# grailbio/bigslice

Hardware: AMD Instinct MI355X
Metric: rows/sec (whole node) Reshuffle+Reduce group-by (higher is better)
Workload: dtype int64; 1 GPU; model=Reshuffle+Reduce group-by-sum (BASELINE config 3), rows_total=125000000, rows_per_gpu=125000000, distinct_keys=1000000, global_batch=125000000, parallelism=dp1, device=cuda:0

## Files before the change

bigslice_amd/csrc/ext.hip:

```cpp

#include <torch/extension.h>

#include <ATen/hip/HIPContext.h>
#include <hip/hip_runtime.h>

#include <vector>

#include "hash_partition.hip"
#include "groupby.hip"
#include "groupby_part.hip"
#include "sort.hip"
#include "radix.hip"
#include "runs.hip"
#include "runs_multi.hip"
#include "vecagg.hip"
#include "strings.hip"
#include "expr.hip"
#include "tokenize.hip"
#include "groupby_multi.hip"

namespace {

#define HIP_CHECK(expr)                                              \
  do {                                                               \
// ... 187 lines not shown
  TORCH_CHECK(cap > 0 && (cap & (cap - 1)) == 0, "capacity must be 2^k");
  TORCH_CHECK(tkeys.is_cuda() && tkeys.is_contiguous() &&
              tkeys.scalar_type() == torch::kInt64);
  for (const auto& tab : tabs)
    TORCH_CHECK(tab.is_cuda() && tab.is_contiguous() &&
                tab.size(0) == cap + 1);
  TORCH_CHECK(flags.is_cuda() && flags.is_contiguous() &&
              flags.scalar_type() == torch::kInt32 && flags.numel() >= 2);
  return cap;
}

uint32_t bucket_shift(int64_t cap, int64_t nbuckets) {
  TORCH_CHECK(cap > 0 && (cap & (cap - 1)) == 0 && cap <= (int64_t(1) << 31),
              "capacity must be 2^k");
  TORCH_CHECK(nbuckets >= 2 && nbuckets <= GBP_MAX_BUCKETS &&
                  (nbuckets & (nbuckets - 1)) == 0 && nbuckets <= cap,
              "nbuckets must be a power of two in [2, ", GBP_MAX_BUCKETS,
              "] and at most the capacity");
  uint32_t shift = 0;
  while ((cap >> shift) > nbuckets) ++shift;
  return shift;
}

void groupby_insert(torch::Tensor keys, std::vector<torch::Tensor> vals,
                    std::vector<int64_t> aggs, torch::Tensor tkeys,
                    std::vector<torch::Tensor> tabs, torch::Tensor flags,
                    int64_t max_probes) {
  TORCH_CHECK(keys.is_cuda() && keys.scalar_type() == torch::kInt64);
  keys = keys.contiguous();
  int64_t n = keys.size(0);
  if (n == 0) return;
  int64_t cap = table_cap(tkeys, tabs, flags);
  ValCols vc = make_val_cols(vals, tabs, aggs);
  int blocks = (int)std::min<int64_t>((n + THREADS - 1) / THREADS, 32768);
  hipLaunchKernelGGL(k_groupby_insert, dim3(blocks), dim3(THREADS), 0,
                     current_stream(), keys.data_ptr<int64_t>(), n, vc,
                     tkeys.data_ptr<int64_t>(), cap, GB_HASH_SEED,
                     flags.data_ptr<int32_t>(),
                     flags.data_ptr<int32_t>() + 1, max_probes);
  HIP_CHECK(hipGetLastError());
}

torch::Tensor slot_pids(torch::Tensor keys, int64_t cap,
                        int64_t nparts) {
  TORCH_CHECK(keys.is_cuda() && keys.scalar_type() == torch::kInt64);
  keys = keys.contiguous();
  int64_t n = keys.size(0);
  auto pids = torch::empty({n}, keys.options().dtype(torch::kInt32));
  int blocks = (int)std::min<int64_t>((n + THREADS - 1) / THREADS, 32768);
  hipLaunchKernelGGL(k_slot_pids, dim3(blocks), dim3(THREADS), 0,
                     current_stream(), keys.data_ptr<int64_t>(), n, cap,
                     (int32_t)nparts, GB_HASH_SEED,
                     pids.data_ptr<int32_t>());
  HIP_CHECK(hipGetLastError());
  return pids;
}

void groupby_insert_lds(torch::Tensor keys, torch::Tensor vals,
                        torch::Tensor tkeys, torch::Tensor tab,
                        torch::Tensor flags, int64_t max_probes,
                        int64_t target_blocks) {
  TORCH_CHECK(keys.is_cuda() && keys.scalar_type() == torch::kInt64);
  TORCH_CHECK(vals.scalar_type() == torch::kInt64);
  keys = keys.contiguous();
  vals = vals.contiguous();
  int64_t n = keys.size(0);
  if (n == 0) return;
  int64_t cap = table_cap(tkeys, {tab}, flags);
  if (target_blocks <= 0) target_blocks = 32768;
  int64_t nblocks = std::min<int64_t>((n + THREADS - 1) / THREADS,
                                      target_blocks);
  int64_t rpb = 0;
  hipLaunchKernelGGL(k_groupby_insert_sum_i64_lds, dim3((uint32_t)nblocks),
                     dim3(THREADS), 0, current_stream(),
                     keys.data_ptr<int64_t>(), vals.data_ptr<int64_t>(), n,
                     tkeys.data_ptr<int64_t>(),
                     (long long*)tab.data_ptr<int64_t>(), cap, GB_HASH_SEED,
                     flags.data_ptr<int32_t>(),
                     flags.data_ptr<int32_t>() + 1, max_probes, rpb,
                     (int32_t)1, (uint32_t*)nullptr);
  HIP_CHECK(hipGetLastError());
}

std::tuple<torch::Tensor, torch::Tensor> part_scatter_impl(
    const torch::Tensor& keys, const torch::Tensor& vals, int64_t cap,
    int64_t nbuckets) {
  int64_t n = keys.size(0);
  TORCH_CHECK(n > 0 && n < (int64_t(1) << 31), "1 <= rows < 2^31");
  const uint32_t shift = bucket_shift(cap, nbuckets);
  const uint32_t seed = GB_HASH_SEED;
  const uint32_t mask = (uint32_t)(cap - 1);
  const uint32_t nb = (uint32_t)nbuckets;
  const int64_t ntiles = (n + GBP_SCATTER_ROWS - 1) / GBP_SCATTER_ROWS;
  auto opts32 = keys.options().dtype(torch::kInt32);
  auto hist = torch::empty({ntiles * nbuckets}, opts32);
  auto totals = torch::empty({nbuckets}, opts32);
  auto pairs = torch::empty({n, 2}, keys.options());
  auto stream = current_stream();
  hipLaunchKernelGGL(k_gbp_hist, dim3((uint32_t)ntiles), dim3(GBP_THREADS),
                     0, stream, keys.data_ptr<int64_t>(), n, nb, seed, mask,
                     shift, (uint32_t*)hist.data_ptr<int32_t>());
  HIP_CHECK(hipGetLastError());
  hipLaunchKernelGGL(k_gbp_offsets, dim3((nb + 63) / 64),
                     dim3(GBP_OFF_THREADS), 0, stream,
                     (uint32_t*)hist.data_ptr<int32_t>(), ntiles, nb,
                     (uint32_t*)totals.data_ptr<int32_t>());
  HIP_CHECK(hipGetLastError());
  const int64_t per_xcd = (ntiles + 7) / 8;
  hipLaunchKernelGGL(k_gbp_scatter, dim3((uint32_t)(8 * per_xcd)),
                     dim3(GBP_THREADS), 0, stream,
                     keys.data_ptr<int64_t>(), vals.data_ptr<int64_t>(), n,
                     ntiles, nb, seed, mask, shift,
                     (const uint32_t*)hist.data_ptr<int32_t>(),
                     (const uint32_t*)totals.data_ptr<int32_t>(),
                     (GbPair*)pairs.data_ptr<int64_t>());
  HIP_CHECK(hipGetLastError());
  return {pairs, totals};
}

void launch_gbp_aggregate(const torch::Tensor& pairs,
                          const torch::Tensor& tkeys,
                          const torch::Tensor& tab,
                          const torch::Tensor& flags, int64_t cap,
                          int64_t max_probes) {
  const int64_t n = pairs.size(0);
  const int64_t ntiles = (n + GBP_TILE_ROWS - 1) / GBP_TILE_ROWS;
  hipLaunchKernelGGL(k_gbp_aggregate, dim3((uint32_t)ntiles),
                     dim3(GBP_THREADS), 0, current_stream(),
                     (const GbPair*)pairs.data_ptr<int64_t>(), n,
                     tkeys.data_ptr<int64_t>(),
                     (long long*)tab.data_ptr<int64_t>(), cap, GB_HASH_SEED,
                     flags.data_ptr<int32_t>(),
                     flags.data_ptr<int32_t>() + 1, max_probes);
  HIP_CHECK(hipGetLastError());
}

torch::Tensor part_owned_impl(const torch::Tensor& pairs,
                              const torch::Tensor& totals,
                              const torch::Tensor& tkeys,
                              const torch::Tensor& tab,
                              const torch::Tensor& flags,
                              int64_t max_probes) {
  const int64_t n = pairs.size(0);
  const int64_t cap = table_cap(tkeys, {tab}, flags);
  const int64_t nbuckets = totals.size(0);
  TORCH_CHECK(n > 0 && n < (int64_t(1) << 31), "1 <= rows < 2^31");
  const uint32_t shift = bucket_shift(cap, nbuckets);
  const int64_t S = cap / nbuckets;
  TORCH_CHECK(S <= GBP_LDS_SLOTS, "owned pass needs capacity / nbuckets <= ",
              GBP_LDS_SLOTS);
  TORCH_CHECK((uintptr_t)tkeys.data_ptr() % 16 == 0 &&
                  (uintptr_t)tab.data_ptr() % 16 == 0,
              "table must be 16-byte aligned");
  const uint32_t nb = (uint32_t)nbuckets;
  const uint32_t seed = GB_HASH_SEED;
  auto clean = torch::empty({nbuckets}, totals.options());
  auto todo = torch::empty({nbuckets, 2}, totals.options());
  auto stream = current_stream();
  HIP_CHECK(hipFuncSetAttribute(
      (const void*)k_gbp_owned, hipFuncAttributeMaxDynamicSharedMemorySize,
      16 * GBP_LDS_SLOTS));
  hipLaunchKernelGGL(k_gbp_owned, dim3(nb), dim3(GBP_THREADS),
                     (size_t)(16 * S), stream,
                     (GbPair*)pairs.data_ptr<int64_t>(), n,
                     (const uint32_t*)totals.data_ptr<int32_t>(), nb,
                     (uint32_t)S, tkeys.data_ptr<int64_t>(),
                     (long long*)tab.data_ptr<int64_t>(), seed, max_probes,
                     (uint32_t*)clean.data_ptr<int32_t>(),
                     (uint2*)todo.data_ptr<int32_t>());
  HIP_CHECK(hipGetLastError());
  const int64_t ntiles = (n + GBP_TILE_ROWS - 1) / GBP_TILE_ROWS;
  hipLaunchKernelGGL(k_gbp_cleanup, dim3((uint32_t)ntiles),
                     dim3(GBP_THREADS), 0, stream,
                     (const GbPair*)pairs.data_ptr<int64_t>(), n,
                     tkeys.data_ptr<int64_t>(),
                     (long long*)tab.data_ptr<int64_t>(), cap, seed,
                     flags.data_ptr<int32_t>(),
                     flags.data_ptr<int32_t>() + 1, max_probes,
                     (const uint2*)todo.data_ptr<int32_t>(), nb, shift);
  HIP_CHECK(hipGetLastError());
  return clean;
}

void groupby_insert_part(torch::Tensor keys, torch::Tensor vals,
                         torch::Tensor tkeys, torch::Tensor tab,
                         torch::Tensor flags, int64_t max_probes,
                         int64_t nbuckets, int64_t owned) {
  TORCH_CHECK(keys.is_cuda() && keys.scalar_type() == torch::kInt64);
  TORCH_CHECK(vals.scalar_type() == torch::kInt64 &&
              vals.size(0) == keys.size(0));
  TORCH_CHECK(tab.scalar_type() == torch::kInt64);
  keys = keys.contiguous();
  vals = vals.contiguous();
  if (keys.size(0) == 0) return;
  int64_t cap = table_cap(tkeys, {tab}, flags);
  auto parts = part_scatter_impl(keys, vals, cap, nbuckets);
  const torch::Tensor& pairs = std::get<0>(parts);
  if (owned)
    part_owned_impl(pairs, std::get<1>(parts), tkeys, tab, flags,
                    max_probes);
  else
    launch_gbp_aggregate(pairs, tkeys, tab, flags, cap, max_probes);
}

std::tuple<torch::Tensor, torch::Tensor> groupby_part_scatter(
    torch::Tensor keys, torch::Tensor vals, int64_t cap,
    int64_t nbuckets) {
  TORCH_CHECK(keys.is_cuda() && keys.scalar_type() == torch::kInt64);
  TORCH_CHECK(vals.scalar_type() == torch::kInt64 &&
              vals.size(0) == keys.size(0));
  return part_scatter_impl(keys.contiguous(), vals.contiguous(), cap,
                           nbuckets);
}

void groupby_part_aggregate(torch::Tensor pairs, torch::Tensor tkeys,
                            torch::Tensor tab, torch::Tensor flags,
                            int64_t max_probes) {
  TORCH_CHECK(pairs.is_cuda() && pairs.scalar_type() == torch::kInt64 &&
              pairs.is_contiguous() && pairs.dim() == 2 &&
              pairs.size(1) == 2);
  if (pairs.size(0) == 0) return;
  TORCH_CHECK(tab.scalar_type() == torch::kInt64);
  launch_gbp_aggregate(pairs, tkeys, tab, flags,
                       table_cap(tkeys, {tab}, flags), max_probes);
}

torch::Tensor groupby_part_owned(torch::Tensor pairs, torch::Tensor totals,
                                 torch::Tensor tkeys, torch::Tensor tab,
                                 torch::Tensor flags, int64_t max_probes) {
  TORCH_CHECK(pairs.is_cuda() && pairs.scalar_type() == torch::kInt64 &&
              pairs.is_contiguous() && pairs.dim() == 2 &&
              pairs.size(1) == 2);
  TORCH_CHECK(totals.is_cuda() && totals.scalar_type() == torch::kInt32 &&
              totals.is_contiguous() && totals.dim() == 1);
  TORCH_CHECK(tab.scalar_type() == torch::kInt64);
  return part_owned_impl(pairs, totals, tkeys, tab, flags, max_probes);
}

std::vector<torch::Tensor> groupby_compact(torch::Tensor tkeys,
                                           std::vector<torch::Tensor> tabs,
                                           torch::Tensor cursor) {
  int64_t cap = tkeys.size(0) - 1;
  CompactCols cc;
  cc.n = (int)tabs.size();
  std::vector<torch::Tensor> out;
  auto out_keys = torch::empty({cap}, tkeys.options());
  out.push_back(out_keys);
  for (size_t c = 0; c < tabs.size(); ++c) {
    out.push_back(torch::empty({cap}, tabs[c].options()));
    cc.tab[c] = {tabs[c].data_ptr(), dtype_code(tabs[c])};
    cc.out[c] = {out[c + 1].data_ptr(), dtype_code(tabs[c])};
  }
  int64_t spb = (cap + 2047) / 2048;
  if (spb < THREADS) spb = THREADS;
  int blocks = (int)((cap + spb - 1) / spb);
  hipLaunchKernelGGL(k_groupby_compact, dim3(blocks), dim3(THREADS), 0,
                     current_stream(), tkeys.data_ptr<int64_t>(), cap, spb,
                     cc, out_keys.data_ptr<int64_t>(),
                     (unsigned long long*)cursor.data_ptr());
  HIP_CHECK(hipGetLastError());
  return out;
}


#define GBM_LAUNCH(kernel, nk, blocks, ...)                              \
  do {                                                                   \
    switch (nk) {                                                        \
      case 2:                                                            \
        hipLaunchKernelGGL(kernel<2>, dim3(blocks), dim3(THREADS), 0,    \
                           current_stream(), __VA_ARGS__);               \
        break;                                                           \
      case 3:                                                            \
        hipLaunchKernelGGL(kernel<3>, dim3(blocks), dim3(THREADS), 0,    \
                           current_stream(), __VA_ARGS__);               \
        break;                                                           \
      case 4:                                                            \
        hipLaunchKernelGGL(kernel<4>, dim3(blocks), dim3(THREADS), 0,    \
                           current_stream(), __VA_ARGS__);               \
        break;                                                           \
      default:                                                           \
        hipLaunchKernelGGL(kernel<0>, dim3(blocks), dim3(THREADS), 0,    \
                           current_stream(), __VA_ARGS__);               \
    }                                                                    \
    HIP_CHECK(hipGetLastError());                                        \
  } while (0)

uint64_t gbm_fp_mask(int64_t fp_bits) {
  TORCH_CHECK(fp_bits >= 1 && fp_bits <= 64, "fp_bits must be in [1, 64]");
  return fp_bits == 64 ? ~uint64_t(0) : (uint64_t(1) << fp_bits) - 1;
}

int64_t gbm_batch_keys(MkCols& kc, const std::vector<torch::Tensor>& keys) {
  TORCH_CHECK(keys.size() >= 2 && (int)keys.size() <= MAX_KEY_COLS,
              "2..", MAX_KEY_COLS, " key columns supported");
  kc.n = (int)keys.size();
// ... 715 lines not shown
    else if (J == 2) launch(k_expr<true, 2>);
    else launch(k_expr<true, 1>);
  } else {
    if (J == 4) launch(k_expr<false, 4>);
    else if (J == 2) launch(k_expr<false, 2>);
    else launch(k_expr<false, 1>);
  }
  HIP_CHECK(hipGetLastError());
  return outs;
}

std::vector<torch::Tensor> tokenize_bytes(torch::Tensor data,
                                          torch::Tensor offsets,
                                          std::vector<uint64_t> mask4,
                                          bool with_rows) {
  TORCH_CHECK(data.is_cuda() && data.is_contiguous() && data.dim() == 1 &&
              data.scalar_type() == torch::kUInt8,
              "tokenize_bytes: contiguous uint8 device data required");
  TORCH_CHECK(offsets.is_cuda() && offsets.is_contiguous() &&
              offsets.dim() == 1 && offsets.size(0) >= 1 &&
              offsets.scalar_type() == torch::kInt64,
              "tokenize_bytes: contiguous int64 device offsets required");
  TORCH_CHECK(mask4.size() == 4, "tokenize_bytes: mask4 has 4 words");
  const int64_t total = data.size(0);
  const int64_t n = offsets.size(0) - 1;
  TORCH_CHECK(total < (1ll << 31),
              "tokenize_bytes: total bytes must be below 2^31");
  TORCH_CHECK(n > 0 || total == 0, "tokenize_bytes: bytes without rows");
  auto i64 = offsets.options();
  if (total == 0) {
    std::vector<torch::Tensor> out = {torch::empty({0}, data.options()),
                                      torch::zeros({1}, i64)};
    if (with_rows) out.push_back(torch::empty({0}, i64));
    return out;
  }
  if (((uintptr_t)data.data_ptr<uint8_t>() & 15) != 0) data = data.clone();
  const TokMask m{mask4[0], mask4[1], mask4[2], mask4[3]};
  auto stream = current_stream();
  const int64_t ntiles = (total + TOK_TILE - 1) / TOK_TILE;
  auto counts = torch::empty({ntiles, 2}, i64.dtype(torch::kInt32));
  hipLaunchKernelGGL(k_tok_count, dim3((int)ntiles), dim3(TOK_BLOCK), 0,
                     stream, data.data_ptr<uint8_t>(), total,
                     offsets.data_ptr<int64_t>(), n, m,
                     (unsigned int*)counts.data_ptr<int32_t>());
  HIP_CHECK(hipGetLastError());
  auto incl = at::cumsum(counts.view(torch::kInt64).flatten(), 0);
  const uint64_t totals = (uint64_t)incl[ntiles - 1].item<int64_t>();
  const int64_t nkept = (int64_t)(totals & 0xFFFFFFFFull);
  const int64_t ntok = (int64_t)(totals >> 32);
  auto out_data = torch::empty({nkept}, data.options());
  auto out_offsets = torch::empty({ntok + 1}, i64);
  torch::Tensor tok_row;
  if (with_rows) tok_row = torch::empty({ntok}, i64);
  hipLaunchKernelGGL(k_tok_write, dim3((int)ntiles), dim3(TOK_BLOCK), 0,
                     stream, data.data_ptr<uint8_t>(), total,
                     offsets.data_ptr<int64_t>(), n, m,
                     (const unsigned int*)incl.data_ptr<int64_t>(), nkept,
                     ntok,
                     out_data.data_ptr<uint8_t>(),
                     out_offsets.data_ptr<int64_t>(),
                     with_rows ? tok_row.data_ptr<int64_t>() : nullptr);
  HIP_CHECK(hipGetLastError());
  std::vector<torch::Tensor> out = {out_data, out_offsets};
  if (with_rows) out.push_back(tok_row);
  return out;
}

}

PYBIND11_MODULE(TORCH_EXTENSION_NAME, m) {
  m.def("hash_columns", &hash_columns, "murmur3 row hash (K3)");
  m.def("hash_partition", &hash_partition,
        "fused hash+histogram+scatter partitioner (K4)");
  m.def("scatter_by_partition", &scatter_by_partition,
        "scatter rows by precomputed partition ids");
  m.def("groupby_insert", &groupby_insert,
        "hash-aggregate insert pass (K9)");
  m.def("groupby_insert_lds", &groupby_insert_lds,
        "two-level LDS+global insert (int64 sum)");
  m.def("groupby_insert_part", &groupby_insert_part,
        "partitioned LDS pre-aggregating insert (single i64 sum)",
        py::arg("keys"), py::arg("vals"), py::arg("tkeys"), py::arg("tab"),
        py::arg("flags"), py::arg("max_probes"), py::arg("nbuckets"),
        py::arg("owned") = 0);
  m.def("groupby_part_owned", &groupby_part_owned,
        "owner + cleanup passes of the partitioned insert; returns clean");
  m.attr("GBP_OWN_LIMIT") = (int64_t)GBP_OWN_LIMIT;
  m.def("groupby_part_scatter", &groupby_part_scatter,
        "bucket scatter of the partitioned insert");
  m.def("groupby_part_aggregate", &groupby_part_aggregate,
        "aggregate pass of the partitioned insert");
  m.attr("GBP_TILE_ROWS") = (int64_t)GBP_TILE_ROWS;
  m.attr("GBP_LDS_SLOTS") = (int64_t)GBP_LDS_SLOTS;
  m.attr("GBP_MAX_BUCKETS") = (int64_t)GBP_MAX_BUCKETS;
  m.def("groupby_compact", &groupby_compact,
        "hash-aggregate table compaction (K9)");
  m.def("groupby_mk_insert", &groupby_mk_insert,
        "multi-column-key hash-aggregate insert: claim + accumulate (K21)",
        py::arg("keys"), py::arg("vals"), py::arg("aggs"), py::arg("tags"),
        py::arg("kcols"), py::arg("tabs"), py::arg("flags"),
        py::arg("max_probes"), py::arg("fp_bits") = 64);
  m.def("groupby_mk_claim", &groupby_mk_claim,
        "launch 1 of groupby_mk_insert; returns the rows' slots");
  m.def("groupby_mk_accum", &groupby_mk_accum,
        "launch 2 of groupby_mk_insert");
  m.def("groupby_mk_fingerprint", &groupby_mk_fingerprint,
        "the tuple fingerprint groupby_mk_insert claims slots by",
        py::arg("keys"), py::arg("fp_bits") = 64);
  m.attr("MAX_KEY_COLS") = (int64_t)MAX_KEY_COLS;
  m.attr("MAX_COLS") = (int64_t)MAX_COLS;
  m.def("agg_identity", &agg_identity, "aggregation identity fill");
  m.def("radix_argsort", &radix_argsort, "device radix argsort (K6)");
  m.def("radix_sort_keys", &radix_sort_keys, "device radix key sort",
        py::arg("keys"), py::arg("probe") = true);
  m.def("runs_sorted", &runs_sorted,
        "run boundaries of sorted keys (K18)");
  m.def("runs_multi", &runs_multi,
        "run boundaries of lexicographically sorted key columns (K22)");
  m.attr("MRUNS_TILE_ROWS") = (int64_t)MRUNS_TILE;
  m.def("lex_searchsorted", &lex_searchsorted,
        "searchsorted over lexicographically sorted tuples (K22)",
        py::arg("sorted_cols"), py::arg("query_cols"),
        py::arg("right") = false);
  m.def("segment_reduce_runs", &segment_reduce_runs,
        "int64 segmented reduce with precomputed runs (K16 fast path)");
  m.def("runs_guard", &runs_guard,
        "(count, max run length) of a runs_sorted result");
  m.def("segment_reduce_sorted", &segment_reduce_sorted,
        "typed reduce-by-key over sorted pairs (K16; deterministic)");
  m.def("hash_bytes", &hash_bytes,
        "murmur3-32 over varlen byte rows (K17, device strings)");
  m.def("hash_bytes64", &hash_bytes64,
        "64-bit two-seed murmur3 dictionary ids (K17)");
  m.def("colsum16", &colsum16,
        "vector-aggregate experiment: [N,16] f32 colsum, VALU vs MFMA");
  m.def("radix_sort_kv", &radix_sort_kv,
        "direct (key, 8-byte value) radix sort");
  m.def("slot_pids", &slot_pids, "table-slot-range partition ids");
  m.def("expr_apply", &expr_apply,
        "fused Map/Filter expression interpreter (K13)");
  m.def("tokenize_bytes", &tokenize_bytes,
        "split BYTES rows into tokens on a delimiter set (K20)");
  m.attr("TOKENIZE_TILE_BYTES") = (int64_t)TOK_TILE;
}
```

bigslice_amd/csrc/groupby_part.hip:

```cpp

#include <hip/hip_runtime.h>

#include "columns.h"

#define GBP_THREADS 512
#define GBP_SCATTER_ROWS 4096
#define GBP_TILE_ROWS 8192
#define GBP_LDS_SLOTS 4096
#define GBP_LDS_BITS 12
#define GBP_LDS_PROBES 8
#define GBP_MAX_BUCKETS 1024

struct __attribute__((aligned(16))) GbPair {
  long long k;
  long long v;
};

__device__ __forceinline__ uint32_t gbp_bucket(long long k, uint32_t seed,
                                               uint32_t mask,
                                               uint32_t shift) {
  if (k == GB_SENTINEL) return 0;
  return (mm3_u64((uint64_t)k, seed) & mask) >> shift;
}

extern "C" __global__ __launch_bounds__(GBP_THREADS) void k_gbp_hist(
    const int64_t* keys, int64_t n, uint32_t nb, uint32_t seed,
    uint32_t mask, uint32_t shift, uint32_t* hist) {
  __shared__ uint32_t lh[GBP_MAX_BUCKETS];
  for (uint32_t b = threadIdx.x; b < nb; b += GBP_THREADS) lh[b] = 0;
  __syncthreads();
  const int64_t base = (int64_t)blockIdx.x * GBP_SCATTER_ROWS;
#pragma unroll
  for (int j = 0; j < GBP_SCATTER_ROWS / GBP_THREADS; ++j) {
    const int64_t i = base + j * GBP_THREADS + threadIdx.x;
    if (i < n) atomicAdd(&lh[gbp_bucket(keys[i], seed, mask, shift)], 1u);
  }
  __syncthreads();
  uint32_t* row = hist + (int64_t)blockIdx.x * nb;
  for (uint32_t b = threadIdx.x; b < nb; b += GBP_THREADS) row[b] = lh[b];
}

#define GBP_OFF_THREADS 1024
#define GBP_OFF_WAVES (GBP_OFF_THREADS / 64)

extern "C" __global__ __launch_bounds__(GBP_OFF_THREADS) void k_gbp_offsets(
    uint32_t* hist, int64_t ntiles, uint32_t nb, uint32_t* totals) {
  __shared__ uint32_t wsum[GBP_OFF_WAVES][64];
  const int lane = threadIdx.x & 63;
  const int w = threadIdx.x >> 6;
  const uint32_t col = blockIdx.x * 64 + lane;
  const bool ok = col < nb;
  const int64_t chunk = (ntiles + GBP_OFF_WAVES - 1) / GBP_OFF_WAVES;
  const int64_t t0 = min((int64_t)w * chunk, ntiles);
  const int64_t t1 = min(t0 + chunk, ntiles);
  uint32_t s = 0;
  if (ok) {
#pragma unroll 8
    for (int64_t t = t0; t < t1; ++t) s += hist[t * nb + col];
  }
  wsum[w][lane] = s;
  __syncthreads();
  uint32_t run = 0;
  for (int w2 = 0; w2 < w; ++w2) run += wsum[w2][lane];
  if (w == GBP_OFF_WAVES - 1 && ok) totals[col] = run + s;
  if (!ok) return;
  int64_t t = t0;
  for (; t + 8 <= t1; t += 8) {
    uint32_t v[8];
#pragma unroll
    for (int j = 0; j < 8; ++j) v[j] = hist[(t + j) * nb + col];
#pragma unroll
    for (int j = 0; j < 8; ++j) {
      hist[(t + j) * nb + col] = run;
      run += v[j];
    }
  }
  for (; t < t1; ++t) {
    const uint32_t v = hist[t * nb + col];
    hist[t * nb + col] = run;
    run += v;
  }
}

__device__ __forceinline__ void gbp_block_scan(uint32_t* a, uint32_t nb,
                                               uint32_t* wtmp) {
  const uint32_t i0 = 2 * threadIdx.x;
  const uint32_t x0 = i0 < nb ? a[i0] : 0;
  const uint32_t x1 = i0 + 1 < nb ? a[i0 + 1] : 0;
  const uint32_t s = x0 + x1;
  const int lane = threadIdx.x & 63;
  const int w = threadIdx.x >> 6;
  uint32_t run = s;
  for (int off = 1; off < 64; off <<= 1) {
    const uint32_t up = __shfl_up(run, off);
    if (lane >= off) run += up;
  }
  if (lane == 63) wtmp[w] = run;
  __syncthreads();
  uint32_t base = 0;
  for (int w2 = 0; w2 < w; ++w2) base += wtmp[w2];
  const uint32_t excl = base + run - s;
  if (i0 < nb) a[i0] = excl;
  if (i0 + 1 < nb) a[i0 + 1] = excl + x0;
  __syncthreads();
}

extern "C" __global__ __launch_bounds__(GBP_THREADS) void k_gbp_scatter(
    const int64_t* keys, const int64_t* vals, int64_t n, int64_t ntiles,
    uint32_t nb, uint32_t seed, uint32_t mask, uint32_t shift,
    const uint32_t* hist, const uint32_t* totals, GbPair* out) {
  __shared__ GbPair stage[GBP_SCATTER_ROWS];
  __shared__ uint32_t lstart[GBP_MAX_BUCKETS];
  __shared__ uint32_t delta[GBP_MAX_BUCKETS];
  __shared__ uint32_t wtmp[GBP_THREADS / 64];
  const int64_t per_xcd = (ntiles + 7) / 8;
  const int64_t tile = (int64_t)(blockIdx.x & 7) * per_xcd + (blockIdx.x >> 3);
  if (tile >= ntiles) return;
  for (uint32_t b = threadIdx.x; b < nb; b += GBP_THREADS) {
    lstart[b] = 0;
    delta[b] = totals[b];
  }
  __syncthreads();
  constexpr int R = GBP_SCATTER_ROWS / GBP_THREADS;
  const int64_t base = tile * GBP_SCATTER_ROWS;
  const uint32_t cnt = (uint32_t)min((int64_t)GBP_SCATTER_ROWS, n - base);
  long long k[R], v[R];
  uint32_t br[R];
#pragma unroll
  for (int j = 0; j < R; ++j) {
    const uint32_t p = j * GBP_THREADS + threadIdx.x;
    if (p < cnt) {
      k[j] = keys[base + p];
      v[j] = vals[base + p];
    }
  }
#pragma unroll
  for (int j = 0; j < R; ++j) {
    const uint32_t p = j * GBP_THREADS + threadIdx.x;
    if (p < cnt) {
      const uint32_t b = gbp_bucket(k[j], seed, mask, shift);
      br[j] = (b << 16) | atomicAdd(&lstart[b], 1u);
    }
  }
  __syncthreads();
  gbp_block_scan(lstart, nb, wtmp);
  gbp_block_scan(delta, nb, wtmp);
#pragma unroll
  for (int j = 0; j < R; ++j) {
    const uint32_t p = j * GBP_THREADS + threadIdx.x;
    if (p < cnt) {
      GbPair pr;
      pr.k = k[j];
      pr.v = v[j];
      stage[lstart[br[j] >> 16] + (br[j] & 0xffffu)] = pr;
    }
  }
  const uint32_t* hrow = hist + tile * nb;
  for (uint32_t b = threadIdx.x; b < nb; b += GBP_THREADS)
    delta[b] += hrow[b] - lstart[b];
  __syncthreads();
  for (uint32_t p = threadIdx.x; p < cnt; p += GBP_THREADS) {
    const GbPair pr = stage[p];
    const uint32_t b = gbp_bucket(pr.k, seed, mask, shift);
    const uint32_t d = delta[b] + p;
    if (d < n) out[d] = pr;
  }
}

__device__ __forceinline__ bool gbp_lds_add(long long k, long long v,
                                            long long* lk, long long* lv,
                                            uint32_t seed) {
  uint32_t h = (mm3_u64((uint64_t)k, seed) * 0x9e3779b1u) >>
               (32 - GBP_LDS_BITS);
  for (int p = 0; p < GBP_LDS_PROBES; ++p) {
    long long cur = lk[h];
    if (cur == GB_SENTINEL) {
      const long long prev = atomicCAS((unsigned long long*)&lk[h],
                                       (unsigned long long)GB_SENTINEL,
                                       (unsigned long long)k);
      cur = (prev == GB_SENTINEL) ? k : prev;
    }
    if (cur == k) {
      atomicAdd((unsigned long long*)&lv[h], (unsigned long long)v);
      return true;
    }
    h = (h + 1) & (GBP_LDS_SLOTS - 1);
  }
  return false;
}

template <bool CLEAN>
__device__ __forceinline__ void gbp_aggregate_tile(
    const GbPair* pairs, int64_t n, int64_t* tkeys, long long* tab,
    int64_t cap, uint32_t seed, int32_t* sentinel_seen, int32_t* overflow,
    int64_t max_probes, const uint2* todo, uint32_t nb, uint32_t shift) {
  __shared__ long long lk[GBP_LDS_SLOTS];
  __shared__ long long lv[GBP_LDS_SLOTS];
  __shared__ uint32_t lend[CLEAN ? GBP_MAX_BUCKETS : 1];
  __shared__ uint32_t hull[2];
  const uint64_t gmask = (uint64_t)cap - 1;
  const int64_t base = (int64_t)blockIdx.x * GBP_TILE_ROWS;
  int64_t first = base, last = n;
  if constexpr (CLEAN) {
    const uint32_t t0 = (uint32_t)base;
    const uint32_t t1 = (uint32_t)min(base + GBP_TILE_ROWS, n);
    if (threadIdx.x == 0) {
      hull[0] = t1;
      hull[1] = t0;
    }
    __syncthreads();
    for (uint32_t b = threadIdx.x; b < nb; b += GBP_THREADS) {
      const uint2 se = todo[b];
      lend[b] = se.y;
      if (se.y > se.x && se.x < t1 && se.y > t0) {
        atomicMin(&hull[0], max(se.x, t0));
        atomicMax(&hull[1], min(se.y, t1));
      }
    }
    __syncthreads();
    first = hull[0];
    last = hull[1];
    if (first >= last) return;
    if (last - first <= GBP_THREADS) {
      const int64_t i = first + threadIdx.x;
      if (i < last) {
        const GbPair pr = pairs[i];
        if (i < (int64_t)lend[gbp_bucket(pr.k, seed, (uint32_t)gmask, shift)])
          gb_global_insert_sum(pr.k, pr.v, tkeys, tab, gmask, cap, seed,
                               sentinel_seen, overflow, max_probes);
      }
      return;
    }
  }
  for (int s = threadIdx.x; s < GBP_LDS_SLOTS; s += GBP_THREADS) {
    lk[s] = GB_SENTINEL;
    lv[s] = 0;
  }
  __syncthreads();
  constexpr int G = 8;
  for (int j0 = 0; j0 < GBP_TILE_ROWS / GBP_THREADS; j0 += G) {
    if (CLEAN && first + j0 * GBP_THREADS >= last) break;
    GbPair pr[G];
#pragma unroll
    for (int j = 0; j < G; ++j) {
      const int64_t i = first + (j0 + j) * GBP_THREADS + threadIdx.x;
      if (i < last) pr[j] = pairs[i];
    }
#pragma unroll
    for (int j = 0; j < G; ++j) {
// ... 171 lines not shown
```

bigslice_amd/kernels/groupby.py:

```python

from __future__ import annotations

import dataclasses
import math
import os
import sys
from typing import List, Optional

import torch

from . import _C, ALLOW_FALLBACK, _require
from .sortedkeys import sort_combine

_AGG_CODES = {"sum": 0, "min": 1, "max": 2, "prod": 3}

_GB_KEY_DTYPES = (torch.int64,)
_GB_VAL_DTYPES = (torch.int64, torch.int32, torch.float32, torch.float64)

GB_SENTINEL = -(1 << 63)
MAX_PROBES = 128

PART_TILE_ROWS = _C.GBP_TILE_ROWS if _C is not None else None
PART_LDS_SLOTS = _C.GBP_LDS_SLOTS if _C is not None else None
PART_MAX_BUCKETS = _C.GBP_MAX_BUCKETS if _C is not None else None

PART_OWN_LIMIT = _C.GBP_OWN_LIMIT if _C is not None else None


@dataclasses.dataclass(frozen=True)
class Options:
    mode: Optional[str] = None
    combine: str = "auto"
    part: bool = True
    part_owned: bool = True
    lds_blocks: int = 4096
    sample_rows: int = 1 << 19
    debug: bool = False

    @classmethod
    def from_env(cls, env=None) -> "Options":
        env = os.environ if env is None else env
        mode = env.get("BIGSLICE_GB_MODE")
        return cls(
            mode=mode if mode in ("lds", "global", "part") else None,
            combine=env.get("BIGSLICE_GB_COMBINE", "auto"),
            part=env.get("BIGSLICE_GB_PART", "1") == "1",
            part_owned=env.get("BIGSLICE_GB_PART_OWNED", "1") == "1",
            lds_blocks=int(env.get("BIGSLICE_GB_LDS_BLOCKS", "4096")),
            sample_rows=int(env.get("BIGSLICE_GB_SAMPLE_ROWS",
                                    str(1 << 19))),
            debug=bool(env.get("BIGSLICE_GB_DEBUG")))


def _next_pow2(n: int) -> int:
    c = 1024
    while c < n:
        c <<= 1
    return c


def part_buckets(n: int, nkeys: float, cap: int,
                 lds_slots: int = PART_LDS_SLOTS,
                 tile_rows: int = PART_TILE_ROWS,
                 max_buckets: int = PART_MAX_BUCKETS) -> int:
    room = lds_slots / 2 - tile_rows * nkeys / max(n, 1)
    b = 2
    while b < max_buckets and (room <= 0 or b * room < nkeys):
        b <<= 1
    return min(b, cap)


def part_owned_buckets(n: int, cap: int, lds_slots: int, tile_rows: int,
                       max_buckets: int):
    want = max(cap / lds_slots, n / tile_rows)
    b = 2
    while b < want:
        b <<= 1
    b = max(2, min(b, max_buckets, cap))
    s = cap // b
    return (b, s) if s <= lds_slots else None


PART_BAND = (6.0, 500.0)


def forced_mode(opts: Options, sum_i64: bool) -> Optional[str]:
    if opts.mode in ("lds", "global"):
        return opts.mode
    if opts.mode == "part" and not sum_i64:
        return "global"
    if opts.combine == "sort":
        return "sort"
    return None


def choose_mode(distinct: int, sample_n: int, batch_n: int, sum_i64: bool,
                opts: Options, cap_hint: Optional[int] = None):
    forced = forced_mode(opts, sum_i64)
    if forced:
        return forced, None, cap_hint
    s = sample_n
    K = None
    if distinct < s:
        K = float(distinct)
        for _ in range(20):
            K = distinct / (1.0 - math.exp(-s / K))
        if cap_hint is None:
            cap_hint = _next_pow2(min(max(int(4 * K), 1024), 1 << 30))
    if distinct * 32 <= s:
        mode = "lds"
    elif distinct * 100 > s * 88:
        mode = "sort"
    else:
        rows_per_key = batch_n / max(K, 1.0)
        mode = "sort" if rows_per_key > 500 else "global"
        if (mode == "global" and sum_i64 and opts.part
                and PART_BAND[0] <= rows_per_key <= PART_BAND[1]):
            mode = "part"
    if opts.mode == "part":
        mode = "part"
    elif mode == "sort" and opts.combine == "hash":
        mode = "global"
    return mode, K, cap_hint


def part_plan(n: int, cap: int, key_estimate: Optional[float],
              opts: Options, lds_slots: int, tile_rows: int,
              max_buckets: int, min_rows: int):
    if not min_rows <= n < (1 << 31):
        return None
# ... 73 lines not shown
                            cap + 1)
            for dt, code in zip(self.val_dtypes, self.codes)]
        self.flags = torch.zeros(2, dtype=torch.int32, device=dev)

    @property
    def _sort_combinable(self) -> bool:
        return (_C is not None
                and str(self.device).startswith("cuda")
                and all(a in ("sum", "min", "max") for a in self.aggs)
                and all(dt in _GB_VAL_DTYPES for dt in self.val_dtypes))

    def _start_sample(self, keys: torch.Tensor) -> None:
        self._sample_forced = forced_mode(self.opts, self._sum_i64)
        if self._sample_forced:
            return
        prefix = min(keys.shape[0], self.opts.sample_rows)
        sk = _C.radix_sort_keys(keys[:prefix].contiguous(),
                                probe=False)
        self._sample_n = prefix
        self._sample_batch_n = keys.shape[0]
        self._sample_ne = (sk[1:] != sk[:-1]).sum()

    def _read_sample(self) -> str:
        if self._sample_forced:
            return self._sample_forced
        distinct = 1 + int(self._sample_ne.item())
        mode, self._key_estimate, self.cap_hint = choose_mode(
            distinct, self._sample_n, self._sample_batch_n, self._sum_i64,
            self.opts, self.cap_hint)
        if self.opts.debug:
            print(f"[gb] sample={self._sample_n} distinct={distinct} "
                  f"cap_hint={self.cap_hint} mode={mode}",
                  file=sys.stderr, flush=True)
        return mode

    def insert(self, keys: torch.Tensor, vals: List[torch.Tensor]):
        n = keys.shape[0]
        if n == 0:
            return
        self.rows += n
        if not self._sort_combinable:
            self._insert_now(keys, vals)
            return
        if self._mode is None:
            if n >= self._SMALL_BATCH:
                self._start_sample(keys)
                self._mode = "pending"
            self._deferred.append((keys, vals))
            return
        if self._mode == "pending":
            self._mode = self._read_sample()
        if self._mode == "sort":
            self._deferred.append((keys, vals))
            return
        self._flush_deferred()
        self._insert_now(keys, vals)

    def _flush_deferred(self):
        pending, self._deferred = self._deferred, []
        for k, v in pending:
            self._insert_now(k, v)

    def _insert_now(self, keys: torch.Tensor, vals: List[torch.Tensor]):
        if self.cap is None:
            from .. import config
            hint = self.cap_hint or min(
                2 * keys.shape[0],
                getattr(config, "GROUPBY_INITIAL_CAP", 1 << 23))
            self._alloc(_next_pow2(hint))
        self.batches.append((keys, vals))
        mode = self._mode if self._sum_i64 else None
        plan = part_plan(
            keys.shape[0], self.cap, self._key_estimate, self.opts,
            PART_LDS_SLOTS, PART_TILE_ROWS, PART_MAX_BUCKETS,
            self._PART_MIN_ROWS) if mode == "part" else None
        if mode == "lds":
            _C.groupby_insert_lds(keys, vals[0], self.tkeys, self.tabs[0],
                                  self.flags, MAX_PROBES,
                                  self.opts.lds_blocks)
        elif plan is not None:
            kind, nbuckets = plan
            _C.groupby_insert_part(keys, vals[0], self.tkeys, self.tabs[0],
                                   self.flags, MAX_PROBES, nbuckets,
                                   *([1] if kind == "owned" else []))
        else:
            _C.groupby_insert(keys, list(vals), self.codes, self.tkeys,
                              self.tabs, self.flags, MAX_PROBES)

    def _finish_deferred(self):
        from ..utils import stats
        if self._mode not in (None, "sort"):
            self._flush_deferred()
            return None
        batches = self._deferred
        keys = (batches[0][0] if len(batches) == 1
                else torch.cat([k for k, _ in batches]))
        if self._mode is None:
            self._start_sample(keys)
            self._mode = self._read_sample()
            if self._mode != "sort":
                self._flush_deferred()
                return None
        self._deferred = []
        vcols = (list(batches[0][1]) if len(batches) == 1
                 else [torch.cat(cols)
                       for cols in zip(*(v for _, v in batches))])
        uk, outs = sort_combine(keys, vcols, self.codes)
        if self.cap is not None:
            self._insert_now(uk, outs)
            return None
        stats.DEFAULT.add("combiner/keys", int(uk.shape[0]))
        return uk, outs

    def finish(self):
        from ..utils import stats
        stats.DEFAULT.add("combiner/records", self.rows)
        if self._mode == "pending":
            self._mode = self._read_sample()
        if self._deferred:
            done = self._finish_deferred()
            if done is not None:
                return done
        if self.cap is None:
            empty = torch.empty(0, dtype=torch.int64, device=self.device)
            return empty, [torch.empty(0, dtype=dt, device=self.device)
                           for dt in self.val_dtypes]
        while True:
            cursor = torch.zeros(1, dtype=torch.int64, device=self.device)
            outs = _C.groupby_compact(self.tkeys, self.tabs, cursor)
            host = torch.cat([cursor,
                              self.flags.to(torch.int64)]).cpu()
            nkeys, sentinel_seen, overflow = (int(host[0]), int(host[1]),
                                              int(host[2]))
            if overflow:
                batches = self.batches
                self._alloc(regrow_capacity(self.cap, self.rows))
                self.batches = []
                for keys, vals in batches:
                    self._insert_now(keys, vals)
                continue
            keys = outs[0][:nkeys]
            vals = [o[:nkeys] for o in outs[1:]]
            if sentinel_seen:
                keys = torch.cat([keys, torch.full(
                    (1,), GB_SENTINEL, dtype=torch.int64,
                    device=self.device)])
                vals = [torch.cat([v, t[self.cap:self.cap + 1]])
                        for v, t in zip(vals, self.tabs)]
            self.batches = []
            stats.DEFAULT.add("combiner/keys", int(keys.shape[0]))
            return keys, vals


def groupby(keys: torch.Tensor, vals: List[torch.Tensor],
            aggs: List[str]):
    t = GroupTable([v.dtype for v in vals], aggs, keys.device)
    t.insert(keys, list(vals))
    return t.finish()
```

Baseline: 27.22 billion rows/sec.

## Process groups of tiles per workgroup in partition histogram and scatter

The histogram and scatter kernels now have each workgroup handle a group of consecutive tiles (up to 8, sized so there are about 512 groups). This shrinks the per-tile histogram array and the offsets scan to one row per group. The scatter keeps running per-bucket bases across the tiles of its group, prefetches the next tile's keys and values into registers, and uses 16-byte vector loads when the inputs are aligned. The cost is fewer workgroups, which lowers parallelism and latency hiding, plus extra LDS scans and barriers for every tile.

```diff
diff --git a/bigslice_amd/csrc/ext.hip b/bigslice_amd/csrc/ext.hip
--- a/bigslice_amd/csrc/ext.hip
+++ b/bigslice_amd/csrc/ext.hip
@@ -293,36 +293,50 @@
   HIP_CHECK(hipGetLastError());
 }
 
+constexpr int64_t GBP_GROUP_WGS = 512;
+constexpr int64_t GBP_MAX_GROUP = 8;
+
+int64_t part_group_tiles(int64_t n) {
+  const int64_t ntiles = (n + GBP_SCATTER_ROWS - 1) / GBP_SCATTER_ROWS;
+  const int64_t g = (ntiles + GBP_GROUP_WGS - 1) / GBP_GROUP_WGS;
+  return std::min(std::max(g, (int64_t)1), GBP_MAX_GROUP);
+}
+
 std::tuple<torch::Tensor, torch::Tensor> part_scatter_impl(
     const torch::Tensor& keys, const torch::Tensor& vals, int64_t cap,
-    int64_t nbuckets) {
+    int64_t nbuckets, int64_t group_tiles) {
   int64_t n = keys.size(0);
   TORCH_CHECK(n > 0 && n < (int64_t(1) << 31), "1 <= rows < 2^31");
+  TORCH_CHECK(group_tiles >= 0 && group_tiles <= 65536,
+              "0 <= group_tiles <= 65536");
   const uint32_t shift = bucket_shift(cap, nbuckets);
   const uint32_t seed = GB_HASH_SEED;
   const uint32_t mask = (uint32_t)(cap - 1);
   const uint32_t nb = (uint32_t)nbuckets;
   const int64_t ntiles = (n + GBP_SCATTER_ROWS - 1) / GBP_SCATTER_ROWS;
+  const int64_t G = group_tiles ? group_tiles : part_group_tiles(n);
+  const int64_t ngroups = (ntiles + G - 1) / G;
   auto opts32 = keys.options().dtype(torch::kInt32);
-  auto hist = torch::empty({ntiles * nbuckets}, opts32);
+  auto gsum = torch::empty({ngroups * nbuckets}, opts32);
   auto totals = torch::empty({nbuckets}, opts32);
   auto pairs = torch::empty({n, 2}, keys.options());
   auto stream = current_stream();
-  hipLaunchKernelGGL(k_gbp_hist, dim3((uint32_t)ntiles), dim3(GBP_THREADS),
-                     0, stream, keys.data_ptr<int64_t>(), n, nb, seed, mask,
-                     shift, (uint32_t*)hist.data_ptr<int32_t>());
+  hipLaunchKernelGGL(k_gbp_hist, dim3((uint32_t)ngroups), dim3(GBP_THREADS),
+                     0, stream, keys.data_ptr<int64_t>(), n, ntiles,
+                     (uint32_t)G, nb, seed, mask, shift,
+                     (uint32_t*)gsum.data_ptr<int32_t>());
   HIP_CHECK(hipGetLastError());
   hipLaunchKernelGGL(k_gbp_offsets, dim3((nb + 63) / 64),
                      dim3(GBP_OFF_THREADS), 0, stream,
-                     (uint32_t*)hist.data_ptr<int32_t>(), ntiles, nb,
+                     (uint32_t*)gsum.data_ptr<int32_t>(), ngroups, nb,
                      (uint32_t*)totals.data_ptr<int32_t>());
   HIP_CHECK(hipGetLastError());
-  const int64_t per_xcd = (ntiles + 7) / 8;
+  const int64_t per_xcd = (ngroups + 7) / 8;
   hipLaunchKernelGGL(k_gbp_scatter, dim3((uint32_t)(8 * per_xcd)),
                      dim3(GBP_THREADS), 0, stream,
                      keys.data_ptr<int64_t>(), vals.data_ptr<int64_t>(), n,
-                     ntiles, nb, seed, mask, shift,
-                     (const uint32_t*)hist.data_ptr<int32_t>(),
+                     ntiles, (uint32_t)G, ngroups, nb, seed, mask, shift,
+                     (const uint32_t*)gsum.data_ptr<int32_t>(),
                      (const uint32_t*)totals.data_ptr<int32_t>(),
                      (GbPair*)pairs.data_ptr<int64_t>());
   HIP_CHECK(hipGetLastError());
@@ -396,7 +410,8 @@
 void groupby_insert_part(torch::Tensor keys, torch::Tensor vals,
                          torch::Tensor tkeys, torch::Tensor tab,
                          torch::Tensor flags, int64_t max_probes,
-                         int64_t nbuckets, int64_t owned) {
+                         int64_t nbuckets, int64_t owned,
+                         int64_t group_tiles) {
   TORCH_CHECK(keys.is_cuda() && keys.scalar_type() == torch::kInt64);
   TORCH_CHECK(vals.scalar_type() == torch::kInt64 &&
               vals.size(0) == keys.size(0));
@@ -405,7 +420,7 @@
   vals = vals.contiguous();
   if (keys.size(0) == 0) return;
   int64_t cap = table_cap(tkeys, {tab}, flags);
-  auto parts = part_scatter_impl(keys, vals, cap, nbuckets);
+  auto parts = part_scatter_impl(keys, vals, cap, nbuckets, group_tiles);
   const torch::Tensor& pairs = std::get<0>(parts);
   if (owned)
     part_owned_impl(pairs, std::get<1>(parts), tkeys, tab, flags,
@@ -416,12 +431,12 @@
 
 std::tuple<torch::Tensor, torch::Tensor> groupby_part_scatter(
     torch::Tensor keys, torch::Tensor vals, int64_t cap,
-    int64_t nbuckets) {
+    int64_t nbuckets, int64_t group_tiles) {
   TORCH_CHECK(keys.is_cuda() && keys.scalar_type() == torch::kInt64);
   TORCH_CHECK(vals.scalar_type() == torch::kInt64 &&
               vals.size(0) == keys.size(0));
   return part_scatter_impl(keys.contiguous(), vals.contiguous(), cap,
-                           nbuckets);
+                           nbuckets, group_tiles);
 }
 
 void groupby_part_aggregate(torch::Tensor pairs, torch::Tensor tkeys,
@@ -1303,12 +1318,17 @@
         "partitioned LDS pre-aggregating insert (single i64 sum)",
         py::arg("keys"), py::arg("vals"), py::arg("tkeys"), py::arg("tab"),
         py::arg("flags"), py::arg("max_probes"), py::arg("nbuckets"),
-        py::arg("owned") = 0);
+        py::arg("owned") = 0, py::arg("group_tiles") = 0);
   m.def("groupby_part_owned", &groupby_part_owned,
         "owner + cleanup passes of the partitioned insert; returns clean");
   m.attr("GBP_OWN_LIMIT") = (int64_t)GBP_OWN_LIMIT;
   m.def("groupby_part_scatter", &groupby_part_scatter,
-        "bucket scatter of the partitioned insert");
+        "bucket scatter of the partitioned insert", py::arg("keys"),
+        py::arg("vals"), py::arg("cap"), py::arg("nbuckets"),
+        py::arg("group_tiles") = 0);
+  m.def("groupby_part_group_tiles", &part_group_tiles,
+        "tiles per group the partitioned insert picks for n rows");
+  m.attr("GBP_SCATTER_ROWS") = (int64_t)GBP_SCATTER_ROWS;
   m.def("groupby_part_aggregate", &groupby_part_aggregate,
         "aggregate pass of the partitioned insert");
   m.attr("GBP_TILE_ROWS") = (int64_t)GBP_TILE_ROWS;
diff --git a/bigslice_amd/csrc/groupby_part.hip b/bigslice_amd/csrc/groupby_part.hip
--- a/bigslice_amd/csrc/groupby_part.hip
+++ b/bigslice_amd/csrc/groupby_part.hip
@@ -23,20 +23,84 @@
   return (mm3_u64((uint64_t)k, seed) & mask) >> shift;
 }
 
+__device__ __forceinline__ void gbp_group_tiles(int64_t g, uint32_t G,
+                                                int64_t ntiles, int64_t* t0,
+                                                int64_t* t1) {
+  *t0 = g * G;
+  *t1 = min(*t0 + (int64_t)G, ntiles);
+}
+
+template <bool WIDE>
+__device__ __forceinline__ uint32_t gbp_row(int j) {
+  return WIDE ? (j >> 1) * 2 * GBP_THREADS + 2 * threadIdx.x + (j & 1)
+              : j * GBP_THREADS + threadIdx.x;
+}
+
+template <bool WIDE, int R>
+__device__ __forceinline__ void gbp_load_rows(const int64_t* col, int64_t r,
+                                              int64_t r1, long long (&x)[R]) {
+  if constexpr (WIDE) {
+#pragma unroll
+    for (int j = 0; j < R; j += 2) {
+      const int64_t i = r + gbp_row<true>(j);
+      if (i + 1 < r1) {
+        const longlong2 two = *(const longlong2*)(col + i);
+        x[j] = two.x;
+        x[j + 1] = two.y;
+      } else if (i < r1) {
+        x[j] = col[i];
+      }
+    }
+  } else {
+#pragma unroll
+    for (int j = 0; j < R; ++j) {
+      const int64_t i = r + gbp_row<false>(j);
+      if (i < r1) x[j] = col[i];
+    }
+  }
+}
+
+#define GBP_HIST_C (GBP_SCATTER_ROWS / GBP_THREADS)
+
+template <bool WIDE>
+__device__ __forceinline__ void gbp_hist_rows(const int64_t* keys, int64_t r0,
+                                              int64_t r1, uint32_t seed,
+                                              uint32_t mask, uint32_t shift,
+                                              uint32_t* lh) {
+  constexpr int64_t CH = (int64_t)GBP_HIST_C * GBP_THREADS;
+  long long k[GBP_HIST_C], kn[GBP_HIST_C];
+  gbp_load_rows<WIDE>(keys, r0, r1, k);
+  __syncthreads();
+  for (int64_t r = r0; r < r1; r += CH) {
+    const bool more = r + CH < r1;
+    if (more) gbp_load_rows<WIDE>(keys, r + CH, r1, kn);
+#pragma unroll
+    for (int j = 0; j < GBP_HIST_C; ++j) {
+      if (r + gbp_row<WIDE>(j) < r1)
+        atomicAdd(&lh[gbp_bucket(k[j], seed, mask, shift)], 1u);
+    }
+    if (more) {
+#pragma unroll
+      for (int j = 0; j < GBP_HIST_C; ++j) k[j] = kn[j];
+    }
+  }
+}
+
 extern "C" __global__ __launch_bounds__(GBP_THREADS) void k_gbp_hist(
-    const int64_t* keys, int64_t n, uint32_t nb, uint32_t seed,
-    uint32_t mask, uint32_t shift, uint32_t* hist) {
+    const int64_t* keys, int64_t n, int64_t ntiles, uint32_t G, uint32_t nb,
+    uint32_t seed, uint32_t mask, uint32_t shift, uint32_t* gsum) {
   __shared__ uint32_t lh[GBP_MAX_BUCKETS];
+  int64_t t0, t1;
+  gbp_group_tiles(blockIdx.x, G, ntiles, &t0, &t1);
+  const int64_t r0 = t0 * GBP_SCATTER_ROWS;
+  const int64_t r1 = min(t1 * GBP_SCATTER_ROWS, n);
   for (uint32_t b = threadIdx.x; b < nb; b += GBP_THREADS) lh[b] = 0;
-  __syncthreads();
-  const int64_t base = (int64_t)blockIdx.x * GBP_SCATTER_ROWS;
-#pragma unroll
-  for (int j = 0; j < GBP_SCATTER_ROWS / GBP_THREADS; ++j) {
-    const int64_t i = base + j * GBP_THREADS + threadIdx.x;
-    if (i < n) atomicAdd(&lh[gbp_bucket(keys[i], seed, mask, shift)], 1u);
-  }
-  __syncthreads();
-  uint32_t* row = hist + (int64_t)blockIdx.x * nb;
+  if (((uintptr_t)keys & 15) == 0)
+    gbp_hist_rows<true>(keys, r0, r1, seed, mask, shift, lh);
+  else
+    gbp_hist_rows<false>(keys, r0, r1, seed, mask, shift, lh);
+  __syncthreads();
+  uint32_t* row = gsum + (int64_t)blockIdx.x * nb;
   for (uint32_t b = threadIdx.x; b < nb; b += GBP_THREADS) row[b] = lh[b];
 }
 
@@ -105,66 +169,133 @@
   __syncthreads();
 }
 
+__device__ __forceinline__ void gbp_tile_scan(uint32_t* lstart,
+                                              uint32_t* delta, uint32_t nb,
+                                              uint32_t* wtmp,
+                                              uint32_t* base0,
+                                              uint32_t* base1) {
+  const uint32_t i0 = 2 * threadIdx.x;
+  const uint32_t x0 = i0 < nb ? lstart[i0] : 0;
+  const uint32_t x1 = i0 + 1 < nb ? lstart[i0 + 1] : 0;
+  const uint32_t s = x0 + x1;
+  const int lane = threadIdx.x & 63;
+  const int w = threadIdx.x >> 6;
+  uint32_t run = s;
+  for (int off = 1; off < 64; off <<= 1) {
+    const uint32_t up = __shfl_up(run, off);
+    if (lane >= off) run += up;
+  }
+  if (lane == 63) wtmp[w] = run;
+  __syncthreads();
+  uint32_t wbase = 0;
+  for (int w2 = 0; w2 < w; ++w2) wbase += wtmp[w2];
+  const uint32_t excl = wbase + run - s;
+  if (i0 < nb) {
+    lstart[i0] = excl;
+    delta[i0] = *base0 - excl;
+    *base0 += x0;
+  }
+  if (i0 + 1 < nb) {
+    lstart[i0 + 1] = excl + x0;
+    delta[i0 + 1] = *base1 - (excl + x0);
+    *base1 += x1;
+  }
+  __syncthreads();
+}
+
+#define GBP_SCATTER_R (GBP_SCATTER_ROWS / GBP_THREADS)
+
+template <bool WIDE>
+__device__ __forceinline__ void gbp_scatter_group(
+    const int64_t* keys, const int64_t* vals, int64_t n, int64_t t0,
+    int64_t t1, uint32_t nb, uint32_t seed, uint32_t mask, uint32_t shift,
+    const uint32_t* grow, const uint32_t* totals, GbPair* out, GbPair* stage,
+    uint32_t* lstart, uint32_t* delta, uint32_t* wtmp) {
+  constexpr int R = GBP_SCATTER_R;
+  long long k[R], v[R], kn[R], vn[R];
+  uint32_t br[R];
+  const uint32_t i0 = 2 * threadIdx.x;
+  const uint2 tot = i0 + 1 < nb ? *(const uint2*)(totals + i0)
+                                : make_uint2(0, 0);
+  const uint2 gs = i0 + 1 < nb ? *(const uint2*)(grow + i0)
+                               : make_uint2(0, 0);
+  gbp_load_rows<WIDE>(keys, t0 * GBP_SCATTER_ROWS, n, k);
+  gbp_load_rows<WIDE>(vals, t0 * GBP_SCATTER_ROWS, n, v);
+  if (i0 + 1 < nb) {
+    lstart[i0] = 0;
+    lstart[i0 + 1] = 0;
+    delta[i0] = tot.x;
+    delta[i0 + 1] = tot.y;
+  }
+  __syncthreads();
+  gbp_block_scan(delta, nb, wtmp);
+  uint32_t base0 = i0 < nb ? delta[i0] + gs.x : 0;
+  uint32_t base1 = i0 + 1 < nb ? delta[i0 + 1] + gs.y : 0;
+  for (int64_t t = t0; t < t1; ++t) {
+    const uint32_t cnt = (uint32_t)min((int64_t)GBP_SCATTER_ROWS,
+                                       n - t * GBP_SCATTER_ROWS);
+    if (t + 1 < t1) {
+      gbp_load_rows<WIDE>(keys, (t + 1) * GBP_SCATTER_ROWS, n, kn);
+      gbp_load_rows<WIDE>(vals, (t + 1) * GBP_SCATTER_ROWS, n, vn);
+    }
+#pragma unroll
+    for (int j = 0; j < R; ++j) {
+      if (gbp_row<WIDE>(j) < cnt) {
+        const uint32_t b = gbp_bucket(k[j], seed, mask, shift);
+        br[j] = (b << 16) | atomicAdd(&lstart[b], 1u);
+      }
+    }
+    __syncthreads();
+    gbp_tile_scan(lstart, delta, nb, wtmp, &base0, &base1);
+#pragma unroll
+    for (int j = 0; j < R; ++j) {
+      if (gbp_row<WIDE>(j) < cnt) {
+        GbPair pr;
+        pr.k = k[j];
+        pr.v = v[j];
+        stage[lstart[br[j] >> 16] + (br[j] & 0xffffu)] = pr;
+      }
+    }
+    __syncthreads();
+    for (uint32_t b = threadIdx.x; b < nb; b += GBP_THREADS) lstart[b] = 0;
+    for (uint32_t p = threadIdx.x; p < cnt; p += GBP_THREADS) {
+      const GbPair pr = stage[p];
+      const uint32_t b = gbp_bucket(pr.k, seed, mask, shift);
+      const uint32_t d = delta[b] + p;
+      if (d < n) out[d] = pr;
+    }
+    if (t + 1 < t1) {
+      __syncthreads();
+#pragma unroll
+      for (int j = 0; j < R; ++j) {
+        k[j] = kn[j];
+        v[j] = vn[j];
+      }
+    }
+  }
+}
+
 extern "C" __global__ __launch_bounds__(GBP_THREADS) void k_gbp_scatter(
     const int64_t* keys, const int64_t* vals, int64_t n, int64_t ntiles,
-    uint32_t nb, uint32_t seed, uint32_t mask, uint32_t shift,
-    const uint32_t* hist, const uint32_t* totals, GbPair* out) {
+    uint32_t G, int64_t ngroups, uint32_t nb, uint32_t seed, uint32_t mask,
+    uint32_t shift, const uint32_t* gsum, const uint32_t* totals,
+    GbPair* out) {
   __shared__ GbPair stage[GBP_SCATTER_ROWS];
   __shared__ uint32_t lstart[GBP_MAX_BUCKETS];
   __shared__ uint32_t delta[GBP_MAX_BUCKETS];
   __shared__ uint32_t wtmp[GBP_THREADS / 64];
-  const int64_t per_xcd = (ntiles + 7) / 8;
-  const int64_t tile = (int64_t)(blockIdx.x & 7) * per_xcd + (blockIdx.x >> 3);
-  if (tile >= ntiles) return;
-  for (uint32_t b = threadIdx.x; b < nb; b += GBP_THREADS) {
-    lstart[b] = 0;
-    delta[b] = totals[b];
-  }
-  __syncthreads();
-  constexpr int R = GBP_SCATTER_ROWS / GBP_THREADS;
-  const int64_t base = tile * GBP_SCATTER_ROWS;
-  const uint32_t cnt = (uint32_t)min((int64_t)GBP_SCATTER_ROWS, n - base);
-  long long k[R], v[R];
-  uint32_t br[R];
-#pragma unroll
-  for (int j = 0; j < R; ++j) {
-    const uint32_t p = j * GBP_THREADS + threadIdx.x;
-    if (p < cnt) {
-      k[j] = keys[base + p];
-      v[j] = vals[base + p];
-    }
-  }
-#pragma unroll
-  for (int j = 0; j < R; ++j) {
-    const uint32_t p = j * GBP_THREADS + threadIdx.x;
-    if (p < cnt) {
-      const uint32_t b = gbp_bucket(k[j], seed, mask, shift);
-      br[j] = (b << 16) | atomicAdd(&lstart[b], 1u);
-    }
-  }
-  __syncthreads();
-  gbp_block_scan(lstart, nb, wtmp);
-  gbp_block_scan(delta, nb, wtmp);
-#pragma unroll
-  for (int j = 0; j < R; ++j) {
-    const uint32_t p = j * GBP_THREADS + threadIdx.x;
-    if (p < cnt) {
-      GbPair pr;
-      pr.k = k[j];
-      pr.v = v[j];
-      stage[lstart[br[j] >> 16] + (br[j] & 0xffffu)] = pr;
-    }
-  }
-  const uint32_t* hrow = hist + tile * nb;
-  for (uint32_t b = threadIdx.x; b < nb; b += GBP_THREADS)
-    delta[b] += hrow[b] - lstart[b];
-  __syncthreads();
-  for (uint32_t p = threadIdx.x; p < cnt; p += GBP_THREADS) {
-    const GbPair pr = stage[p];
-    const uint32_t b = gbp_bucket(pr.k, seed, mask, shift);
-    const uint32_t d = delta[b] + p;
-    if (d < n) out[d] = pr;
-  }
+  const int64_t per_xcd = (ngroups + 7) / 8;
+  const int64_t g = (int64_t)(blockIdx.x & 7) * per_xcd + (blockIdx.x >> 3);
+  if (g >= ngroups) return;
+  int64_t t0, t1;
+  gbp_group_tiles(g, G, ntiles, &t0, &t1);
+  const uint32_t* grow = gsum + g * nb;
+  if ((((uintptr_t)keys | (uintptr_t)vals) & 15) == 0)
+    gbp_scatter_group<true>(keys, vals, n, t0, t1, nb, seed, mask, shift,
+                            grow, totals, out, stage, lstart, delta, wtmp);
+  else
+    gbp_scatter_group<false>(keys, vals, n, t0, t1, nb, seed, mask, shift,
+                             grow, totals, out, stage, lstart, delta, wtmp);
 }
 
 __device__ __forceinline__ bool gbp_lds_add(long long k, long long v,
diff --git a/bigslice_amd/kernels/groupby.py b/bigslice_amd/kernels/groupby.py
--- a/bigslice_amd/kernels/groupby.py
+++ b/bigslice_amd/kernels/groupby.py
@@ -33,6 +33,7 @@
     combine: str = "auto"
     part: bool = True
     part_owned: bool = True
+    part_group: int = 0
     lds_blocks: int = 4096
     sample_rows: int = 1 << 19
     debug: bool = False
@@ -46,6 +47,7 @@
             combine=env.get("BIGSLICE_GB_COMBINE", "auto"),
             part=env.get("BIGSLICE_GB_PART", "1") == "1",
             part_owned=env.get("BIGSLICE_GB_PART_OWNED", "1") == "1",
+            part_group=int(env.get("BIGSLICE_GB_PART_GROUP", "0")),
             lds_blocks=int(env.get("BIGSLICE_GB_LDS_BLOCKS", "4096")),
             sample_rows=int(env.get("BIGSLICE_GB_SAMPLE_ROWS",
                                     str(1 << 19))),
@@ -285,7 +287,8 @@
             kind, nbuckets = plan
             _C.groupby_insert_part(keys, vals[0], self.tkeys, self.tabs[0],
                                    self.flags, MAX_PROBES, nbuckets,
-                                   *([1] if kind == "owned" else []))
+                                   1 if kind == "owned" else 0,
+                                   self.opts.part_group)
         else:
             _C.groupby_insert(keys, list(vals), self.codes, self.tkeys,
                               self.tabs, self.flags, MAX_PROBES)
```

New measurement: 28.58 billion rows/sec, median of 6. 5.0% higher.
